# Nehliin/vortex

Measured on AMD Instinct MI355X. Metric: GiB/s SHA-1 piece hashing (device-resident), 256 KiB pieces, 1/2/4/8 MI355X, higher is better.
Workload: dtype u32; 1 GPU; 65536 x 256 KiB pieces per GPU (BASELINE config 2; config 4 at N=8), SHA-1 + verify vs expected table; pieces_per_gpu=65536, piece_len=262144, parallelism=piece-index shard x1, parity_checked=65536, parity_bit_exact=64881

## Files before the change

### include/vx_tuning.h

```cpp
#ifndef VX_TUNING_H
#define VX_TUNING_H
#include <stddef.h>
#include <stdint.h>
#ifndef VX_MERKLE_ASYNC_FUSED
#define VX_MERKLE_ASYNC_FUSED 1
#endif

#ifdef __cplusplus
extern "C" {
#endif

int vx_sha1_device_ragged_variant(const void* d_base, const uint64_t* d_offsets, const uint32_t* d_lens,
                                  const uint32_t* d_order, uint32_t n, void* d_digests, const void* d_expected,
                                  void* d_matched, void* stream, int variant);
struct vx_ctx;
struct vx_split;
int vx_tuning_zero_copy_plan(uint32_t n, uint64_t total_len);
int vx_tuning_zero_copy_kernel(const uint64_t* d_srcs, const uint32_t* d_lens, uint32_t n, void* d_digests,
                               const void* d_expected, void* d_matched, int loader, void* stream);
int vx_tuning_zero_tail_kernel(const void* d_base, const uint64_t* d_tail_offs, const uint32_t* d_lens,
                               const uint32_t* d_pads, uint32_t n, uint64_t piece_length, const uint32_t* d_states,
                               void* d_digests, void* stream);
int vx_tuning_chunk_kernel(const void* d_base, const uint64_t* d_offsets, const uint32_t* d_lens, uint32_t n,
                           const uint32_t* d_pids, const uint64_t* d_poffs, const uint64_t* d_tlens,
                           uint32_t* d_states, void* d_digests, void* stream);
void vx_tuning_fail_submit_after(struct vx_ctx* ctx, int64_t k);
void vx_tuning_fail_launch_after(struct vx_ctx* ctx, int64_t k);
void vx_tuning_verify_copy_stream(struct vx_ctx* ctx, int mode);
void vx_tuning_stage_huge(struct vx_ctx* ctx, int on);
void vx_tuning_split_rules(struct vx_ctx* ctx, int one_round, uint64_t round_cap, int lag, int learn);
int vx_tuning_plan_ragged(uint32_t n, uint32_t max_len, uint64_t total_len);
size_t vx_tuning_chunk_schedule(uint64_t L, uint64_t C, int head, int tail, uint64_t* out, size_t max);
uint64_t vx_tuning_split_take_tail(struct vx_split* s, uint64_t k, uint64_t* was);
size_t vx_tuning_last_split(const struct vx_ctx* ctx, double* out, size_t max);

int vx_sha1_device_uniform_variant(const void* d_base, uint64_t stride, uint32_t len, uint32_t n, void* d_digests,
                                   const void* d_expected, void* d_matched, void* stream, int variant);

int vx_tuning_clock_stamp(void* d_out, uint32_t blocks, void* stream);
int vx_tuning_wall_clock_khz(int device);
int vx_tuning_device_identity(int device, char* bus_id, size_t len, char* uuid16);

#ifdef __cplusplus
}
#endif
#endif
```

### vortex_amd/_lib.py

```python
from __future__ import annotations

import ctypes
import os
import threading

_HERE = os.path.dirname(os.path.abspath(__file__))
LIB_PATH = os.path.join(_HERE, "libvortex_amd.so")
TUNING_PATH = os.path.join(_HERE, "libvortex_amd_tuning.so")

VX_OK = 0
VX_EINVAL = -22
VX_ENOMEM = -12
VX_ERANGE = -34
VX_ENODEV = -19
VX_EDEVICE = -5
VX_EBUSY = -16

VX_MERKLE_BLOCK = 16384
VX_SHA256_LEN = 32

EXPORTS = (
    "vx_abi_version", "vx_last_error", "vx_strerror", "vx_device_count", "vx_config_default",
    "vx_create", "vx_destroy", "vx_register_host_buffer", "vx_unregister_host_buffer",
    "vx_submit", "vx_flush", "vx_poll", "vx_drain", "vx_pending", "vx_set_piece_table", "vx_submit_piece",
    "vx_sha1_batch", "vx_verify_batch", "vx_verify_files", "vx_verify_files_range", "vx_verify_files_multi",
    "vx_sha1_device_uniform", "vx_sha1_device_ragged", "vx_sha1_device_ragged_hint", "vx_sort_order",
    "vx_plan_verify", "vx_plan_verify_gpus", "vx_plan_verify_split", "vx_get_stats", "vx_reset_stats",
    "vx_last_verify", "vx_last_verify_rounds",
    "vx_split_init", "vx_split_claim", "vx_split_done", "vx_split_boundary", "vx_verify_files_split",
    "vx_verify_files_split_multi",
    "vx_merkle_device_uniform", "vx_merkle_device_ragged", "vx_merkle_device_root", "vx_merkle_pad_hash",
    "vx_merkle_verify_batch",
    "vx_merkle_device_blocks", "vx_merkle_device_nodes", "vx_merkle_verify_files", "vx_merkle_verify_files_range",
    "vx_merkle_device_pieces", "vx_merkle_submit", "vx_merkle_poll",
    "vx_merkle_layers_plan", "vx_merkle_device_layers", "vx_merkle_device_proofs", "vx_merkle_verify_layers",
    "vx_merkle_verify_proofs",
    "vx_hybrid_device_pieces", "vx_hybrid_verify_files", "vx_hybrid_verify_files_range",
    "vx_hybrid_submit", "vx_hybrid_set_piece_tables", "vx_hybrid_submit_piece", "vx_hybrid_poll",
)
TUNING_EXPORTS = (
    "vx_synth_fill", "vx_sha1_device_uniform_variant", "vx_sha1_device_ragged_variant",
    "vx_tuning_zero_copy_plan", "vx_tuning_zero_copy_kernel", "vx_tuning_plan_ragged", "vx_tuning_chunk_schedule",
    "vx_tuning_fail_submit_after", "vx_tuning_fail_launch_after", "vx_tuning_verify_copy_stream", "vx_tuning_stage_huge",
    "vx_tuning_split_rules", "vx_tuning_clock_stamp",
    "vx_tuning_wall_clock_khz", "vx_tuning_device_identity", "vx_tuning_split_take_tail",
    "vx_tuning_last_split", "vx_tuning_zero_tail_kernel", "vx_tuning_chunk_kernel",
)


class VxError(RuntimeError):
    def __init__(self, code: int, where: str, msg: str):
        super().__init__(f"{where} failed: {code} ({msg})")
        self.code = code
        self.refused = None


class vx_completion(ctypes.Structure):
    _fields_ = [("tag", ctypes.c_uint64), ("matched", ctypes.c_uint8), ("digest", ctypes.c_uint8 * 20),
                ("_pad", ctypes.c_uint8 * 3)]


class vx_merkle_completion(ctypes.Structure):
    _fields_ = [("tag", ctypes.c_uint64), ("matched", ctypes.c_uint8), ("root", ctypes.c_uint8 * 32),
                ("_pad", ctypes.c_uint8 * 7)]


class vx_hybrid_completion(ctypes.Structure):
    _fields_ = [("tag", ctypes.c_uint64), ("matched", ctypes.c_uint8), ("_pad", ctypes.c_uint8 * 3),
                ("sha1", ctypes.c_uint8 * 20), ("root", ctypes.c_uint8 * 32)]


VX_MERKLE_TILE_ROWS = 512


class vx_merkle_tile(ctypes.Structure):
    _fields_ = [("in_row", ctypes.c_uint32), ("out", ctypes.c_uint32), ("rows", ctypes.c_uint16),
                ("levels", ctypes.c_uint8), ("last", ctypes.c_uint8), ("_pad", ctypes.c_uint32)]


class vx_merkle_layers_plan(ctypes.Structure):
    _fields_ = [("n_layers", ctypes.c_uint32), ("passes", ctypes.c_uint32), ("rows", ctypes.c_uint64),
                ("work_rows", ctypes.c_uint64), ("n_tiles", ctypes.c_uint32), ("pass_tiles", ctypes.c_uint32 * 4),
                ("_pad", ctypes.c_uint32)]


class vx_merkle_proof(ctypes.Structure):
    _fields_ = [("pos", ctypes.c_uint64), ("row", ctypes.c_uint32), ("expected", ctypes.c_uint32),
                ("span", ctypes.c_uint16), ("uncles", ctypes.c_uint8), ("_pad", ctypes.c_uint8 * 5)]


def proof_array(proofs):
    arr = (vx_merkle_proof * max(len(proofs), 1))()
    widths = (64, 32, 32, 16, 8)
    for i, p in enumerate(proofs):
        v = (p.pos, p.row, p.expected, p.span, p.uncles) if isinstance(p, vx_merkle_proof) else tuple(int(x) for x in p)
        if len(v) != 5 or any(not 0 <= x < 1 << w for x, w in zip(v, widths)):
            raise ValueError(f"proof {i}: (pos, row, expected, span, uncles) = {v} does not fit vx_merkle_proof")
        arr[i].pos, arr[i].row, arr[i].expected, arr[i].span, arr[i].uncles = v
    return arr


ABI_VERSION = 3

CONFIG_OPTIONS = ("zero_copy", "direct_io", "batch_chunk", "verify_chunk", "verify_cold_chunk", "verify_ramp",
                  "refuse_when_full")


class vx_config(ctypes.Structure):
    _fields_ = [("device", ctypes.c_int32), ("max_piece_len", ctypes.c_uint32), ("batch_pieces", ctypes.c_uint32),
                ("slots", ctypes.c_uint32), ("slot_bytes", ctypes.c_uint64)] + \
        [(name, ctypes.c_uint32) for name in CONFIG_OPTIONS]


class vx_plan(ctypes.Structure):
    _fields_ = [("gpu_s", ctypes.c_double), ("gpu_chain_s", ctypes.c_double), ("gpu_transfer_s", ctypes.c_double),
                ("cpu_s", ctypes.c_double), ("piece_latency_s", ctypes.c_double),
                ("cpu_piece_latency_s", ctypes.c_double), ("use_gpu", ctypes.c_int32), ("_pad", ctypes.c_uint32)]


VX_STATS_HIST = 24


class vx_stats(ctypes.Structure):
    _fields_ = [(name, ctypes.c_uint64) for name in (
        "pieces_completed", "pieces_mismatched", "bytes_completed", "batches", "chunk_rounds", "gather_tiles",
        "staged_bytes", "io_errors", "submit_stall_ns", "batch_latency_count", "batch_latency_sum_us",
        "batch_latency_max_us")] + [("batch_latency_hist", ctypes.c_uint64 * VX_STATS_HIST)] + [
        (name, ctypes.c_uint64) for name in ("zero_copy_slots", "zero_copy_loader_slots", "submits_refused")]


class vx_verify_trace(ctypes.Structure):
    _fields_ = [(name, ctypes.c_double) for name in (
        "wall_ms", "read_busy_ms", "read_span_ms", "first_read_ms", "copy_busy_ms", "copy_span_ms", "tail_ms")] + [
        ("read_bytes", ctypes.c_uint64), ("copy_bytes", ctypes.c_uint64), ("readers", ctypes.c_uint32),
        ("rounds", ctypes.c_uint32), ("direct_bytes", ctypes.c_uint64),
        ("chunk_bytes", ctypes.c_uint64)]


VX_ROUND_NEW_WINDOW, VX_ROUND_HEAD_RAMP, VX_ROUND_TAIL_RAMP = 1, 2, 4


class vx_verify_round(ctypes.Structure):
    _fields_ = [(name, ctypes.c_double) for name in (
        "read_submit_ms", "read_done_ms", "enqueue_ms", "copy_start_ms", "copy_end_ms", "kernel_end_ms")] + [
        ("bytes", ctypes.c_uint64), ("offset", ctypes.c_uint64), ("lanes", ctypes.c_uint32),
        ("flags", ctypes.c_uint32)]


class vx_split(ctypes.Structure):
    _fields_ = [("word", ctypes.c_uint64), ("pool_done", ctypes.c_uint64), ("start_ns", ctypes.c_uint64),
                ("first", ctypes.c_uint64), ("end", ctypes.c_uint64), ("cpu_threads", ctypes.c_uint32),
                ("engines", ctypes.c_uint32), ("cpu_thread_rate", ctypes.c_double),
                ("pool_last_ns", ctypes.c_uint64)]


_lib = None
_tuning = None
_lock = threading.Lock()


def _declare(L: ctypes.CDLL, tuning: bool = False) -> None:
    c = ctypes
    vp = c.c_void_p
    sig = {
        "vx_abi_version": ([], c.c_int),
        "vx_last_error": ([], c.c_char_p),
        "vx_strerror": ([c.c_int], c.c_char_p),
        "vx_device_count": ([], c.c_int),
        "vx_config_default": ([c.POINTER(vx_config), c.c_uint32], None),
        "vx_create": ([c.POINTER(vx_config), c.POINTER(vp)], c.c_int),
        "vx_destroy": ([vp], c.c_int),
        "vx_register_host_buffer": ([vp, vp, c.c_size_t], c.c_int),
        "vx_unregister_host_buffer": ([vp, vp], c.c_int),
        "vx_submit": ([vp, c.c_uint64, vp, c.c_uint32, vp], c.c_int),
        "vx_flush": ([vp], c.c_int),
        "vx_set_piece_table": ([vp, vp, c.c_uint32], c.c_int),
        "vx_submit_piece": ([vp, c.c_uint64, vp, c.c_uint32, c.c_uint32], c.c_int),
        "vx_poll": ([vp, c.POINTER(vx_completion), c.c_size_t], c.c_int64),
        "vx_drain": ([vp, c.c_uint32], c.c_int),
        "vx_pending": ([vp], c.c_uint64),
        "vx_get_stats": ([vp, c.POINTER(vx_stats)], c.c_int),
        "vx_reset_stats": ([vp], c.c_int),
        "vx_sha1_batch": ([vp, vp, vp, c.c_size_t, vp], c.c_int),
        "vx_verify_batch": ([vp, vp, vp, vp, c.c_size_t, vp, vp], c.c_int),
        "vx_verify_files": ([vp, vp, vp, c.c_size_t, c.c_uint32, vp, c.c_size_t, vp, c.c_uint32], c.c_int64),
        "vx_verify_files_range": ([vp, vp, vp, c.c_size_t, c.c_uint32, vp, c.c_size_t, c.c_size_t, c.c_size_t, vp,
                                   c.c_uint32], c.c_int64),
        "vx_verify_files_multi": ([vp, c.c_size_t, vp, vp, c.c_size_t, c.c_uint32, vp, c.c_size_t, vp, c.c_uint32],
                                  c.c_int64),
        "vx_sha1_device_uniform": ([vp, c.c_uint64, c.c_uint32, c.c_uint32, vp, vp, vp, vp], c.c_int),
        "vx_sha1_device_ragged": ([vp, vp, vp, vp, c.c_uint32, vp, vp, vp, vp], c.c_int),
        "vx_sha1_device_ragged_hint": ([vp, vp, vp, vp, c.c_uint32, c.c_uint32, c.c_uint64, vp, vp, vp, vp],
                                       c.c_int),
        "vx_sort_order": ([vp, c.c_uint32, vp], c.c_int),
        "vx_last_verify": ([vp, c.POINTER(vx_verify_trace)], c.c_int),
        "vx_last_verify_rounds": ([vp, c.POINTER(vx_verify_round), c.c_size_t], c.c_int64),
        "vx_plan_verify": ([c.c_uint64, c.c_uint32, c.c_uint64, c.c_uint32, c.c_double, c.POINTER(vx_plan)], c.c_int),
        "vx_plan_verify_gpus": ([c.c_uint64, c.c_uint32, c.c_uint64, c.c_uint32, c.c_double, c.c_uint32,
                                 c.POINTER(vx_plan)], c.c_int),
        "vx_plan_verify_split": ([c.c_uint64, c.c_uint32, c.c_uint64, c.c_uint32, c.c_double, c.c_uint32,
                                  c.POINTER(c.c_uint64), c.POINTER(c.c_uint64), c.POINTER(vx_plan)], c.c_int),
        "vx_split_init": ([c.POINTER(vx_split), c.c_uint64, c.c_uint64, c.c_uint32, c.c_double], c.c_int),
        "vx_split_claim": ([c.POINTER(vx_split)], c.c_int64),
        "vx_split_done": ([c.POINTER(vx_split), c.c_uint64], None),
        "vx_split_boundary": ([c.POINTER(vx_split)], c.c_uint64),
        "vx_verify_files_split": ([vp, vp, vp, c.c_size_t, c.c_uint32, vp, c.c_size_t, c.POINTER(vx_split), vp,
                                   c.c_uint32], c.c_int64),
        "vx_verify_files_split_multi": ([vp, c.c_size_t, vp, vp, c.c_size_t, c.c_uint32, vp, c.c_size_t,
                                         c.POINTER(vx_split), vp, c.c_uint32], c.c_int64),
        "vx_merkle_device_uniform": ([vp, c.c_uint64, c.c_uint32, c.c_uint32, c.c_uint32, c.c_uint32, vp, vp, vp, vp,
                                      vp], c.c_int),
        "vx_merkle_device_ragged": ([vp, vp, vp, vp, c.c_uint32, c.c_uint32, vp, vp, vp, vp, vp], c.c_int),
        "vx_merkle_device_root": ([vp, c.c_uint32, c.c_uint32, vp, vp, vp], c.c_int),
        "vx_merkle_pad_hash": ([c.c_uint32, vp], c.c_int),
        "vx_merkle_verify_batch": ([vp, vp, vp, vp, c.c_size_t, c.c_uint32, vp, vp, vp], c.c_int),
        "vx_merkle_device_blocks": ([vp, vp, vp, c.c_uint32, vp, vp], c.c_int),
        "vx_merkle_device_nodes": ([vp, vp, c.c_uint32, c.c_uint32, vp, vp, vp, vp], c.c_int),
        "vx_merkle_verify_files": ([vp, vp, vp, c.c_size_t, c.c_uint32, vp, c.c_size_t, vp, c.c_uint32], c.c_int64),
        "vx_merkle_verify_files_range": ([vp, vp, vp, c.c_size_t, c.c_uint32, vp, c.c_size_t, c.c_size_t,
                                          c.c_size_t, vp, c.c_uint32], c.c_int64),
        "vx_merkle_device_pieces": ([vp, vp, vp, vp, c.c_uint32, c.c_uint32, vp, vp, vp, vp, vp], c.c_int),
        "vx_merkle_submit": ([vp, c.c_uint64, vp, c.c_uint32, c.c_uint32, vp], c.c_int),
        "vx_merkle_poll": ([vp, c.POINTER(vx_merkle_completion), c.c_size_t], c.c_int64),
        "vx_merkle_layers_plan": ([vp, c.c_uint32, c.POINTER(vx_merkle_layers_plan), vp, c.c_size_t], c.c_int),
        "vx_merkle_device_layers": ([vp, c.POINTER(vx_merkle_layers_plan), vp, c.c_uint32, vp, vp, vp, vp, vp],
                                    c.c_int),
        "vx_merkle_device_proofs": ([vp, vp, c.c_uint32, vp, vp, vp, vp], c.c_int),
        "vx_merkle_verify_layers": ([vp, vp, vp, c.c_uint32, c.c_uint32, vp, vp, vp], c.c_int),
        "vx_merkle_verify_proofs": ([vp, vp, c.c_uint64, vp, c.c_uint32, vp, c.c_uint32, vp, vp], c.c_int),
        "vx_hybrid_device_pieces": ([vp, vp, vp, vp, vp, c.c_uint32, c.c_uint32, vp, vp, vp, vp, vp, vp, vp], c.c_int),
        "vx_hybrid_verify_files": ([vp, vp, vp, c.c_size_t, c.c_uint32, vp, vp, c.c_size_t, vp, c.c_uint32],
                                   c.c_int64),
        "vx_hybrid_verify_files_range": ([vp, vp, vp, c.c_size_t, c.c_uint32, vp, vp, c.c_size_t, c.c_size_t,
                                          c.c_size_t, vp, c.c_uint32], c.c_int64),
        "vx_hybrid_submit": ([vp, c.c_uint64, vp, c.c_uint32, c.c_uint32, c.c_uint32, vp, vp], c.c_int),
        "vx_hybrid_set_piece_tables": ([vp, vp, vp, c.c_uint32], c.c_int),
        "vx_hybrid_submit_piece": ([vp, c.c_uint64, vp, c.c_uint32, c.c_uint32, c.c_uint32, c.c_uint32], c.c_int),
        "vx_hybrid_poll": ([vp, c.POINTER(vx_hybrid_completion), c.c_size_t], c.c_int64),
    }
    if tuning:
        sig.update({
            "vx_sha1_device_uniform_variant": ([vp, c.c_uint64, c.c_uint32, c.c_uint32, vp, vp, vp, vp, c.c_int],
                                               c.c_int),
            "vx_sha1_device_ragged_variant": ([vp, vp, vp, vp, c.c_uint32, vp, vp, vp, vp, c.c_int], c.c_int),
            "vx_tuning_zero_copy_plan": ([c.c_uint32, c.c_uint64], c.c_int),
            "vx_tuning_zero_copy_kernel": ([vp, vp, c.c_uint32, vp, vp, vp, c.c_int, vp], c.c_int),
            "vx_tuning_zero_tail_kernel": ([vp, vp, vp, vp, c.c_uint32, c.c_uint64, vp, vp, vp], c.c_int),
            "vx_tuning_chunk_kernel": ([vp, vp, vp, c.c_uint32, vp, vp, vp, vp, vp, vp], c.c_int),
            "vx_tuning_fail_submit_after": ([vp, c.c_int64], None),
            "vx_tuning_fail_launch_after": ([vp, c.c_int64], None),
            "vx_tuning_verify_copy_stream": ([vp, c.c_int], None),
            "vx_tuning_stage_huge": ([vp, c.c_int], None),
            "vx_tuning_split_rules": ([vp, c.c_int, c.c_uint64, c.c_int, c.c_int], None),
            "vx_tuning_clock_stamp": ([vp, c.c_uint32, vp], c.c_int),
            "vx_tuning_wall_clock_khz": ([c.c_int], c.c_int),
            "vx_tuning_device_identity": ([c.c_int, c.c_char_p, c.c_size_t, c.c_char_p], c.c_int),
            "vx_tuning_plan_ragged": ([c.c_uint32, c.c_uint32, c.c_uint64], c.c_int),
            "vx_tuning_split_take_tail": ([c.POINTER(vx_split), c.c_uint64, c.POINTER(c.c_uint64)], c.c_uint64),
            "vx_tuning_last_split": ([vp, c.POINTER(c.c_double), c.c_size_t], c.c_size_t),
            "vx_tuning_chunk_schedule": ([c.c_uint64, c.c_uint64, c.c_int, c.c_int, c.POINTER(c.c_uint64),
                                          c.c_size_t], c.c_size_t),
            "vx_synth_fill": ([vp, c.c_uint64, c.c_uint32, c.c_uint32, c.c_uint64, c.c_uint64, c.c_uint32, vp],
                              c.c_int),
        })
    for name, (args, res) in sig.items():
        fn = getattr(L, name)
        fn.argtypes = args
        fn.restype = res


def _load(path: str, tuning: bool) -> ctypes.CDLL:
    import torch

    if not os.path.exists(path):
        raise ImportError(
            f"{path} is missing: the HIP engine is not built. Run "
            "`python -c 'import __graft_entry__ as g; g.build()'` (or `make -C vortex_amd/csrc`).")
    L = ctypes.CDLL(path)
    _declare(L, tuning)
    if L.vx_abi_version() != ABI_VERSION:
        raise ImportError(f"{os.path.basename(path)} ABI version mismatch")
    return L


def lib() -> ctypes.CDLL:
    global _lib
    if _lib is not None:
        return _lib
    with _lock:
        if _lib is None:
            _lib = _load(LIB_PATH, False)
    return _lib


def tuning() -> ctypes.CDLL:
    global _tuning
    if _tuning is not None:
        return _tuning
    with _lock:
        if _tuning is None:
            _tuning = _load(TUNING_PATH, True)
    return _tuning


def check(rc: int, where: str, L: ctypes.CDLL | None = None) -> int:
    if rc < 0:
        msg = (L or lib()).vx_last_error().decode(errors="replace")
        raise VxError(rc, where, msg)
    return rc
```

### vortex_amd/csrc/sha1_kernels.hip

```cpp
#include <hip/hip_runtime.h>

#include <algorithm>
#include <cstdlib>
#include <stdint.h>

#include "sha1_consumer_asm.inc"
#include "sha1_device.hpp"
#include "vx_kernels.h"

namespace vx {

__device__ __attribute__((aligned(128))) uint4 g_zero_line[32];

__device__ __forceinline__ void load_group(uint4 (&dst)[8], const uint4* src) {
#pragma unroll
    for (int k = 0; k < 8; ++k) dst[k] = src[k];
}

__device__ __forceinline__ void load_group_ordered(uint4 (&dst)[8], const uint4* src) {
    __builtin_amdgcn_sched_barrier(0);
#pragma unroll
    for (int k = 0; k < 4; ++k) dst[k] = src[k];
    __builtin_amdgcn_sched_barrier(0);
#pragma unroll
    for (int k = 4; k < 8; ++k) dst[k] = src[k];
    __builtin_amdgcn_sched_barrier(0);
}

__device__ __forceinline__ void compress_group(State& s, const uint4 (&g)[8]) {
    compress_le(s, g[0], g[1], g[2], g[3]);
    compress_le(s, g[4], g[5], g[6], g[7]);
}

template <int R, bool kUniform, bool kFence = false>
__device__ __forceinline__ void stream_groups(State& s, const uint4* src, uint32_t ng, uint32_t ng_wave) {
    if (ng_wave == 0) return;
    const uint4* base = ng ? src : g_zero_line;
    const uint32_t last = ng ? ng - 1 : 0;
    uint4 ring[R][8];
#pragma unroll
    for (int r = 0; r < R - 1; ++r) {
        const uint32_t g = (uint32_t)r < last ? (uint32_t)r : last;
        if (kFence && kUniform)
            load_group_ordered(ring[r], base + (size_t)g * 8);
        else
            load_group(ring[r], base + (size_t)g * 8);
    }
    if (kFence && kUniform) {
        uint32_t g0 = 0;
        for (; g0 + R <= ng_wave; g0 += R) {
#pragma unroll
            for (int r = 0; r < R; ++r) {
                const uint32_t gl_raw = g0 + r + R - 1;
                const uint32_t gl = gl_raw < last ? gl_raw : last;
                load_group_ordered(ring[(r + R - 1) % R], base + (size_t)gl * 8);
                compress_group(s, ring[r]);
            }
        }
#pragma unroll
        for (int r = 0; r < R - 1; ++r)
            if (g0 + r < ng_wave) compress_group(s, ring[r]);
        return;
    }
    for (uint32_t g0 = 0; g0 < ng_wave; g0 += R) {
#pragma unroll
        for (int r = 0; r < R; ++r) {
            const uint32_t gl_raw = g0 + r + R - 1;
            const uint32_t gl = gl_raw < last ? gl_raw : last;
            load_group(ring[(r + R - 1) % R], base + (size_t)gl * 8);
            if (kUniform) {
                if (g0 + r < ng_wave) compress_group(s, ring[r]);
            } else {
                if (g0 + r < ng) compress_group(s, ring[r]);
            }
        }
    }
}

template <bool kUniform, int R = kRing, bool kFence = false>
__device__ __forceinline__ void hash_piece(State& s, const uint8_t* p, uint32_t len, uint32_t ng_wave) {
    const uint32_t nfull = len >> 6;
    const uint32_t ng = nfull >> 1;
    stream_groups<R, kUniform, kFence>(s, reinterpret_cast<const uint4*>(p), ng, ng_wave);
    const uint8_t* q = p + (size_t)ng * 128;
    if (nfull & 1) {
        const uint4* q4 = reinterpret_cast<const uint4*>(q);
        compress_le(s, q4[0], q4[1], q4[2], q4[3]);
        q += 64;
    }
    finalize(s, q, len & 63u, len);
}

__device__ __forceinline__ void emit(const State& s, uint32_t idx, uint8_t* __restrict__ digests,
                                     const uint8_t* __restrict__ expected, uint8_t* __restrict__ matched,
                                     const uint32_t* __restrict__ exp_index = nullptr) {
    const uint32_t d0 = bswap(s.h0), d1 = bswap(s.h1), d2 = bswap(s.h2), d3 = bswap(s.h3), d4 = bswap(s.h4);
    if (digests) {
        uint32_t* o = reinterpret_cast<uint32_t*>(digests + (size_t)idx * 20);
        o[0] = d0;
        o[1] = d1;
        o[2] = d2;
        o[3] = d3;
        o[4] = d4;
    }
    if (expected && matched) {
        const uint32_t row = exp_index ? exp_index[idx] : idx;
        const uint32_t* x = reinterpret_cast<const uint32_t*>(expected + (size_t)row * 20);
        const bool ok = (x[0] == d0) & (x[1] == d1) & (x[2] == d2) & (x[3] == d3) & (x[4] == d4);
        matched[idx] = ok ? 1 : 0;
    }
}

__device__ __forceinline__ uint32_t wave_min(uint32_t v) {
#pragma unroll
    for (int o = 32; o > 0; o >>= 1) {
        const uint32_t u = __shfl_xor(v, o, 64);
        v = u < v ? u : v;
    }
    return v;
}

__device__ __forceinline__ uint32_t wave_max(uint32_t v) {
#pragma unroll
    for (int o = 32; o > 0; o >>= 1) {
        const uint32_t u = __shfl_xor(v, o, 64);
        v = u > v ? u : v;
    }
    return v;
}

template <int R, bool kAlias = false, bool kFence = false>
__global__ __launch_bounds__(kBlock) void sha1_uniform_kernel(const uint8_t* __restrict__ base, uint64_t stride,
                                                              uint32_t len, uint32_t n,
                                                              uint8_t* __restrict__ digests,
                                                              const uint8_t* __restrict__ expected,
                                                              uint8_t* __restrict__ matched,
                                                              const uint32_t* __restrict__ exp_index) {
    const uint32_t i = blockIdx.x * kBlock + threadIdx.x;
    const uint32_t pi = kAlias ? 0 : (i < n ? i : n - 1);
    State s = iv();
    hash_piece<true, R, kFence>(s, base + (size_t)pi * stride, len, (len >> 7));
    if (i < n) emit(s, i, digests, expected, matched, exp_index);
}

__global__ __launch_bounds__(kBlock) void sha1_ragged_kernel(const uint8_t* __restrict__ base,
                                                             const uint64_t* __restrict__ offsets,
                                                             const uint32_t* __restrict__ lens,
                                                             const uint32_t* __restrict__ order, uint32_t n,
                                                             uint8_t* __restrict__ digests,
                                                             const uint8_t* __restrict__ expected,
                                                             uint8_t* __restrict__ matched,
                                                             const uint32_t* __restrict__ exp_index) {
    const uint32_t j = blockIdx.x * kBlock + threadIdx.x;
    const uint32_t jj = j < n ? j : n - 1;
    const uint32_t idx = order ? order[jj] : jj;
    const uint32_t len = lens[idx];
    const uint8_t* p = base + offsets[idx];
    const uint32_t ng_wave = __builtin_amdgcn_readfirstlane(wave_max(len >> 7));
    State s = iv();
    hash_piece<false>(s, p, len, ng_wave);
    if (j < n) emit(s, idx, digests, expected, matched, exp_index);
}



__device__ __forceinline__ void expand_store(uint32_t (&w)[16], uint4 (*dst)[64], int lane) {
#pragma unroll
    for (int q = 0; q < 4; ++q) dst[q][lane] = make_uint4(w[4 * q], w[4 * q + 1], w[4 * q + 2], w[4 * q + 3]);
#pragma unroll
    for (int q = 4; q < 20; ++q) {
        uint32_t v[4];
#pragma unroll
        for (int j = 0; j < 4; ++j) {
            const int t = 4 * q + j;
            const uint32_t x = rotl(VX_XOR2(VX_PAR(w[(t - 3) & 15], w[(t - 8) & 15], w[(t - 14) & 15]), w[t & 15]), 1);
            w[t & 15] = x;
            v[j] = x;
        }
        dst[q][lane] = make_uint4(v[0], v[1], v[2], v[3]);
    }
}

__device__ __forceinline__ void rounds_lds(State& s, const uint4 (*src)[64], int lane) {
    uint32_t a = s.h0, b = s.h1, c = s.h2, d = s.h3, e = s.h4;
#pragma unroll
    for (int q = 0; q < 20; ++q) {
        const uint4 w4 = src[q][lane];
        const uint32_t wq[4] = {w4.x, w4.y, w4.z, w4.w};
#pragma unroll
        for (int j = 0; j < 4; ++j) {
            const int t = 4 * q + j;
            uint32_t f, k;
            if (t < 20) {
                f = VX_CH(b, c, d);
                k = kK0;
            } else if (t < 40) {
                f = VX_PAR(b, c, d);
                k = kK1;
            } else if (t < 60) {
                f = VX_MAJ(b, c, d);
                k = kK2;
            } else {
                f = VX_PAR(b, c, d);
                k = kK3;
            }
            const uint32_t tmp = rotl(a, 5) + f + e + k + wq[j];
            e = d;
            d = c;
            c = rotl(b, 30);
            b = a;
            a = tmp;
        }
    }
    s.h0 += a;
    s.h1 += b;
    s.h2 += c;
    s.h3 += d;
    s.h4 += e;
}

template <int S>
struct RingLds {
    uint4 w[S][20][64];
};

template <int S>
__device__ __forceinline__ uint32_t ring_slot(uint32_t b) {
    return S == 2 ? (b & 1u) : (b % 3u);
}

template <int S>
__device__ __forceinline__ void publish(uint32_t b) {
    if (S == 2 || b >= 1) __syncthreads();
}

template <int S>
__device__ __forceinline__ void producer_done(uint32_t nb_wave) {
    if (S == 2) {
        __syncthreads();
    } else if (nb_wave) {
        __syncthreads();
        __syncthreads();
    }
}

__device__ __forceinline__ void load_w(uint4 (&r)[20], const uint4 (*src)[64], int lane) {
#pragma unroll
    for (int q = 0; q < 20; ++q) r[q] = src[q][lane];
}

__device__ __forceinline__ void rounds_regs(State& s, const uint4 (&w)[20]) {
    uint32_t a = s.h0, b = s.h1, c = s.h2, d = s.h3, e = s.h4;
#pragma unroll
    for (int q = 0; q < 20; ++q) {
        const uint32_t wq[4] = {w[q].x, w[q].y, w[q].z, w[q].w};
#pragma unroll
        for (int j = 0; j < 4; ++j) {
            const int t = 4 * q + j;
            uint32_t f, k;
            if (t < 20) {
                f = VX_CH(b, c, d);
                k = kK0;
            } else if (t < 40) {
                f = VX_PAR(b, c, d);
                k = kK1;
            } else if (t < 60) {
                f = VX_MAJ(b, c, d);
                k = kK2;
            } else {
                f = VX_PAR(b, c, d);
                k = kK3;
            }
            const uint32_t tmp = rotl(a, 5) + f + e + k + wq[j];
            e = d;
            d = c;
            c = rotl(b, 30);
            b = a;
            a = tmp;
        }
    }
    s.h0 += a;
    s.h1 += b;
    s.h2 += c;
    s.h3 += d;
    s.h4 += e;
}

template <bool kSelect>
__device__ __forceinline__ void consume_asm(State& s, const uint4* lds_lane, uint32_t nb_wave, uint32_t b1,
                                            uint32_t nb) {
    const uint32_t addr = (uint32_t)(uintptr_t)lds_lane;
    if (kSelect)
        asm volatile(VX_CONSUMER_SELECT_ASM
                     : "+v"(s.h0), "+v"(s.h1), "+v"(s.h2), "+v"(s.h3), "+v"(s.h4)
                     : "v"(addr), "s"(nb_wave), "s"(b1), "v"(nb)
                     : VX_CONSUMER_SELECT_ASM_CLOBBERS, "memory");
    else
        asm volatile(VX_CONSUMER_ASM
                     : "+v"(s.h0), "+v"(s.h1), "+v"(s.h2), "+v"(s.h3), "+v"(s.h4)
                     : "v"(addr), "s"(nb_wave), "s"(b1), "v"(nb)
                     : VX_CONSUMER_ASM_CLOBBERS, "memory");
}

template <int S, bool kSelect>
__device__ __forceinline__ void consume(State& s, RingLds<S>& lds, int lane, uint32_t nb_wave, uint32_t b1,
                                        uint32_t nb) {
    if (S == 2) {
        __syncthreads();
        for (uint32_t b = 0; b < b1; ++b) {
            rounds_lds(s, lds.w[b & 1], lane);
            __syncthreads();
        }
        if (kSelect) {
            for (uint32_t b = b1; b < nb_wave; ++b) {
                State t = s;
                rounds_lds(t, lds.w[b & 1], lane);
                if (b < nb) s = t;
                __syncthreads();
            }
        }
        return;
    }
#ifndef VX_CONSUMER_CC
    if (S == 3) {
        consume_asm<kSelect>(s, &lds.w[0][0][lane], nb_wave, b1, nb);
        return;
    }
#endif
    if (nb_wave == 0) return;
    auto step = [&](uint32_t b, const uint4 (&r)[20]) {
        if (!kSelect || b < b1) {
            rounds_regs(s, r);
        } else {
            State t = s;
            rounds_regs(t, r);
            if (b < nb) s = t;
        }
        asm volatile("" : "+v"(s.h0), "+v"(s.h1), "+v"(s.h2), "+v"(s.h3), "+v"(s.h4));
    };
    uint4 r0[20], r1[20];
    __syncthreads();
    load_w(r0, lds.w[0], lane);
    __builtin_amdgcn_s_waitcnt(0xC07F);
    uint32_t b = 0;
    for (; b + 2 <= nb_wave; b += 2) {
        load_w(r1, lds.w[ring_slot<S>(b + 1)], lane);
        __builtin_amdgcn_sched_barrier(0);
        step(b, r0);
        __builtin_amdgcn_sched_barrier(0);
        __syncthreads();
        if (b + 2 < nb_wave) load_w(r0, lds.w[ring_slot<S>(b + 2)], lane);
        __builtin_amdgcn_sched_barrier(0);
        step(b + 1, r1);
        __builtin_amdgcn_sched_barrier(0);
        __syncthreads();
    }
    if (b < nb_wave) {
        step(b, r0);
        __builtin_amdgcn_sched_barrier(0);
        __syncthreads();
    }
}

__device__ __forceinline__ void le_words(uint32_t (&w)[16], const uint4& q0, const uint4& q1, const uint4& q2,
                                         const uint4& q3) {
    const uint4 q[4] = {q0, q1, q2, q3};
#pragma unroll
    for (int k = 0; k < 4; ++k) {
        w[4 * k + 0] = bswap(q[k].x);
        w[4 * k + 1] = bswap(q[k].y);
        w[4 * k + 2] = bswap(q[k].z);
        w[4 * k + 3] = bswap(q[k].w);
    }
}

__device__ __forceinline__ void tail_words(uint32_t (&w)[16], const uint8_t* q, uint32_t rem) {
    const uint32_t* q32 = reinterpret_cast<const uint32_t*>(q);
#pragma unroll
    for (int k = 0; k < 16; ++k) {
        const uint32_t off = 4u * k;
        uint32_t v = 0;
        if (off + 4 <= rem) {
            v = q32[k];
        } else if (off < rem) {
            for (uint32_t j = 0; off + j < rem; ++j) v |= (uint32_t)q[off + j] << (8 * j);
        }
        if (rem >= off && rem < off + 4) v |= 0x80u << (8 * (rem - off));
        w[k] = bswap(v);
    }
}

template <int S>
__global__ __launch_bounds__(kPairBlock) void sha1_split_kernel(const uint8_t* __restrict__ base, uint64_t stride,
                                                                uint32_t len, uint32_t n,
                                                                uint8_t* __restrict__ digests,
                                                                const uint8_t* __restrict__ expected,
                                                                uint8_t* __restrict__ matched,
                                                                const uint32_t* __restrict__ exp_index) {
    __shared__ RingLds<S> lds;
    const int lane = threadIdx.x & 63;
    const int wave = __builtin_amdgcn_readfirstlane(threadIdx.x >> 6);
    const uint32_t i = blockIdx.x * 64 + lane;
    const uint32_t pi = i < n ? i : n - 1;
    const uint8_t* p = base + (size_t)pi * stride;
    const uint32_t nfull = len >> 6;
    const uint32_t rem = len & 63u;
    const uint32_t nb = nfull + (rem <= 55 ? 1u : 2u);

    if (wave == 1) {
        uint32_t b = 0;
        uint32_t w[16];
        const uint32_t ng = len >> 7;
        const uint4* src = reinterpret_cast<const uint4*>(p);
        if (ng) {
            constexpr int R = kRing;
            const uint32_t last = ng - 1;
            uint4 ring[R][8];
#pragma unroll
            for (int r = 0; r < R - 1; ++r) {
                const uint32_t g = (uint32_t)r < last ? (uint32_t)r : last;
                load_group(ring[r], src + (size_t)g * 8);
            }
            for (uint32_t g0 = 0; g0 < ng; g0 += R) {
#pragma unroll
                for (int r = 0; r < R; ++r) {
                    const uint32_t gl_raw = g0 + r + R - 1;
                    const uint32_t gl = gl_raw < last ? gl_raw : last;
                    load_group(ring[(r + R - 1) % R], src + (size_t)gl * 8);
                    if (g0 + r < ng) {
                        le_words(w, ring[r][0], ring[r][1], ring[r][2], ring[r][3]);
                        expand_store(w, lds.w[ring_slot<S>(b)], lane);
                        publish<S>(b);
                        ++b;
                        le_words(w, ring[r][4], ring[r][5], ring[r][6], ring[r][7]);
                        expand_store(w, lds.w[ring_slot<S>(b)], lane);
                        publish<S>(b);
                        ++b;
                    }
                }
            }
        }
        const uint8_t* q = p + (size_t)ng * 128;
        if (nfull & 1) {
            const uint4* q4 = reinterpret_cast<const uint4*>(q);
            le_words(w, q4[0], q4[1], q4[2], q4[3]);
            expand_store(w, lds.w[ring_slot<S>(b)], lane);
            publish<S>(b);
            ++b;
            q += 64;
        }
        tail_words(w, q, rem);
        const uint32_t bits_hi = (uint32_t)(((uint64_t)len * 8u) >> 32);
        const uint32_t bits_lo = (uint32_t)((uint64_t)len * 8u);
        if (rem <= 55) {
            w[14] = bits_hi;
            w[15] = bits_lo;
            expand_store(w, lds.w[ring_slot<S>(b)], lane);
            publish<S>(b);
        } else {
            expand_store(w, lds.w[ring_slot<S>(b)], lane);
            publish<S>(b);
            ++b;
#pragma unroll
            for (int k = 0; k < 14; ++k) w[k] = 0;
            w[14] = bits_hi;
            w[15] = bits_lo;
            expand_store(w, lds.w[ring_slot<S>(b)], lane);
            publish<S>(b);
        }
        producer_done<S>(nb);
    } else {
        State s = iv();
        consume<S, false>(s, lds, lane, nb, nb, nb);
        if (i < n) emit(s, i, digests, expected, matched, exp_index);
    }
}

template <int S>
hipError_t launch_uniform_split_s(const uint8_t* base, uint64_t stride, uint32_t len, uint32_t n, uint8_t* digests,
                                  const uint8_t* expected, uint8_t* matched, hipStream_t stream,
                                  const uint32_t* exp_index) {
    const uint32_t blocks = (n + 63) / 64;
    hipLaunchKernelGGL(sha1_split_kernel<S>, dim3(blocks), dim3(kPairBlock), 0, stream, base, stride, len, n,
                       digests, expected, matched, exp_index);
    return hipGetLastError();
}

hipError_t launch_uniform_split(const uint8_t* base, uint64_t stride, uint32_t len, uint32_t n, uint8_t* digests,
                                const uint8_t* expected, uint8_t* matched, hipStream_t stream,
                                const uint32_t* exp_index) {
    return launch_uniform_split_s<kSplitSlots>(base, stride, len, n, digests, expected, matched, stream, exp_index);
}


constexpr int kBlockRing = 6;

__device__ __forceinline__ void load_block(uint4 (&dst)[4], const uint4* src) {
#pragma unroll
    for (int k = 0; k < 4; ++k) dst[k] = src[k];
}

__device__ __forceinline__ void pad_words(uint32_t (&w)[16], const uint8_t* q, uint32_t rem, uint64_t len,
                                          uint32_t k) {
    const uint32_t bits_hi = (uint32_t)((len * 8u) >> 32);
    const uint32_t bits_lo = (uint32_t)(len * 8u);
    if (k == 0) {
        tail_words(w, q, rem);
        if (rem <= 55) {
            w[14] = bits_hi;
            w[15] = bits_lo;
        }
    } else {
#pragma unroll
        for (int j = 0; j < 16; ++j) w[j] = 0;
        if (k == 1 && rem > 55) {
            w[14] = bits_hi;
            w[15] = bits_lo;
        }
    }
}

template <bool kChunked, int S>
__global__ __launch_bounds__(kPairBlock) void sha1_ragged_split_kernel(
    const uint8_t* __restrict__ base, const uint64_t* __restrict__ offsets, const uint32_t* __restrict__ lens,
    const uint32_t* __restrict__ order, uint32_t n, uint8_t* __restrict__ digests,
    const uint8_t* __restrict__ expected, uint8_t* __restrict__ matched, const uint32_t* __restrict__ exp_index,
    const uint32_t* __restrict__ pids, const uint64_t* __restrict__ poffs, const uint64_t* __restrict__ tlens,
    uint32_t* __restrict__ states) {
    __shared__ RingLds<S> lds;
    const int lane = threadIdx.x & 63;
    const int wave = __builtin_amdgcn_readfirstlane(threadIdx.x >> 6);
    const uint32_t j = blockIdx.x * 64 + lane;
    const uint32_t jj = j < n ? j : n - 1;
    const uint32_t idx = order ? order[jj] : jj;
    const uint32_t len = lens[idx];
    const uint8_t* p = base + offsets[idx];
    const uint32_t pid = kChunked ? pids[idx] : idx;
    const uint64_t poff = kChunked ? poffs[idx] : 0;
    const uint64_t tlen = kChunked ? tlens[idx] : len;
    const bool final_chunk = poff + len == tlen;
    const uint32_t nfull = len >> 6;
    const uint32_t rem = len & 63u;
    const uint32_t nb = final_chunk ? nfull + (rem <= 55 ? 1u : 2u) : nfull;
    const uint32_t nb_wave = __builtin_amdgcn_readfirstlane(wave_max(nb));
    constexpr int R = kBlockRing;
    const uint32_t nfull_min = __builtin_amdgcn_readfirstlane(wave_min(nfull));
    const uint32_t b1 = nfull_min / R * R;

    if (wave == 1) {
        const uint4* src = nfull ? reinterpret_cast<const uint4*>(p) : g_zero_line;
        const uint32_t last = nfull ? nfull - 1 : 0;
        const uint8_t* q = p + (size_t)nfull * 64;
        uint32_t w[16];
        if (b1) {
            uint4 ring[R][4];
#pragma unroll
            for (int r = 0; r < R - 1; ++r) {
                __builtin_amdgcn_sched_barrier(0);
                load_block(ring[r], src + (size_t)r * 4);
            }
            for (uint32_t b0 = 0; b0 < b1; b0 += R) {
#pragma unroll
                for (int r = 0; r < R; ++r) {
                    const uint32_t bl_raw = b0 + r + R - 1;
                    const uint32_t bl = bl_raw < last ? bl_raw : last;
                    __builtin_amdgcn_sched_barrier(0);
                    load_block(ring[(r + R - 1) % R], src + (size_t)bl * 4);
                    __builtin_amdgcn_sched_barrier(0);
                    le_words(w, ring[r][0], ring[r][1], ring[r][2], ring[r][3]);
                    expand_store(w, lds.w[ring_slot<S>(b0 + r)], lane);
                    publish<S>(b0 + r);
                }
            }
        }
        if (b1 < nb_wave) {
            uint32_t padw[16];
            tail_words(padw, q, rem);
            const uint32_t bits_hi = (uint32_t)((tlen * 8u) >> 32);
            const uint32_t bits_lo = (uint32_t)(tlen * 8u);
            if (rem <= 55) {
                padw[14] = bits_hi;
                padw[15] = bits_lo;
            }
            uint4 ring[R][4];
#pragma unroll
            for (int r = 0; r < R - 1; ++r) {
                const uint32_t bl_raw = b1 + r;
                const uint32_t bl = bl_raw < last ? bl_raw : last;
                __builtin_amdgcn_sched_barrier(0);
                load_block(ring[r], src + (size_t)bl * 4);
            }
            for (uint32_t b0 = b1; b0 < nb_wave; b0 += R) {
#pragma unroll
                for (int r = 0; r < R; ++r) {
                    const uint32_t b = b0 + r;
                    const uint32_t bl_raw = b + R - 1;
                    const uint32_t bl = bl_raw < last ? bl_raw : last;
                    __builtin_amdgcn_sched_barrier(0);
                    load_block(ring[(r + R - 1) % R], src + (size_t)bl * 4);
                    __builtin_amdgcn_sched_barrier(0);
                    if (b < nb_wave) {
                        le_words(w, ring[r][0], ring[r][1], ring[r][2], ring[r][3]);
                        const bool is_pad0 = b == nfull;
                        const bool is_pad1 = b == nfull + 1;
#pragma unroll
                        for (int k = 0; k < 16; ++k) {
                            uint32_t v = b < nfull ? w[k] : 0u;
                            v = is_pad0 ? padw[k] : v;
                            if (k >= 14) v = (is_pad1 && rem > 55) ? (k == 14 ? bits_hi : bits_lo) : v;
                            w[k] = v;
                        }
                        expand_store(w, lds.w[ring_slot<S>(b)], lane);
                        publish<S>(b);
                    }
                }
            }
        }
        producer_done<S>(nb_wave);
    } else {
        State s = iv();
        if (kChunked && poff != 0) {
            const uint32_t* st = states + (size_t)pid * 5;
            s = State{st[0], st[1], st[2], st[3], st[4]};
        }
        consume<S, true>(s, lds, lane, nb_wave, b1, nb);
        if (j < n) {
            if (!kChunked || final_chunk) {
                emit(s, pid, digests, expected, matched, exp_index);
            } else {
                uint32_t* st = states + (size_t)pid * 5;
                st[0] = s.h0;
                st[1] = s.h1;
                st[2] = s.h2;
                st[3] = s.h3;
                st[4] = s.h4;
            }
        }
    }
}

constexpr uint32_t kWidePadLds = 40 * 1024;

template <int S>
hipError_t launch_ragged_split_s(const uint8_t* base, const uint64_t* offsets, const uint32_t* lens,
                                 const uint32_t* order, uint32_t n, uint8_t* digests, const uint8_t* expected,
                                 uint8_t* matched, hipStream_t stream, const uint32_t* exp_index,
                                 bool wide = false) {
    const uint32_t blocks = (n + 63) / 64;
    hipLaunchKernelGGL((sha1_ragged_split_kernel<false, S>), dim3(blocks), dim3(kPairBlock),
                       wide ? kWidePadLds : 0u, stream, base,
                       offsets, lens, order, n, digests, expected, matched, exp_index, nullptr, nullptr, nullptr,
                       nullptr);
    return hipGetLastError();
}

hipError_t launch_ragged_split(const uint8_t* base, const uint64_t* offsets, const uint32_t* lens,
                               const uint32_t* order, uint32_t n, uint8_t* digests, const uint8_t* expected,
                               uint8_t* matched, hipStream_t stream, const uint32_t* exp_index) {
    return launch_ragged_split_s<kSplitSlots>(base, offsets, lens, order, n, digests, expected, matched, stream,
                                              exp_index);
}

hipError_t launch_chunk(const uint8_t* base, const uint64_t* offsets, const uint32_t* lens, uint32_t n,
                        const uint32_t* pids, const uint64_t* poffs, const uint64_t* tlens, uint32_t* states,
                        uint8_t* digests, const uint8_t* expected, uint8_t* matched, hipStream_t stream) {
    if (n == 0) return hipSuccess;
    const uint32_t blocks = (n + 63) / 64;
    hipLaunchKernelGGL((sha1_ragged_split_kernel<true, kSplitSlots>), dim3(blocks), dim3(kPairBlock), 0, stream, base, offsets,
                       lens, nullptr, n, digests, expected, matched, nullptr, pids, poffs, tlens, states);
    return hipGetLastError();
}

constexpr uint32_t kZcPieces = 32;
constexpr uint32_t kZcTileBlocks = 8;
constexpr uint32_t kZcChunks = kZcTileBlocks * 4;

typedef uint32_t U32x4 __attribute__((ext_vector_type(4)));
typedef const __attribute__((address_space(1))) U32x4 GlobalU32x4;

__device__ __forceinline__ uint4 zc_load(int k, const uint64_t (&zb)[8], const uint32_t (&zl)[8], uint32_t t) {
    const uint32_t o = t * (kZcTileBlocks * 64) + (k >= 8 ? 256u : 0u);
    const uint64_t zero = reinterpret_cast<uint64_t>(g_zero_line);
    const uint64_t a = (o < zl[k & 7] ? zb[k & 7] + t * (kZcTileBlocks * 64) : zero) + (k >= 8 ? 256u : 0u);
    const U32x4 v = *reinterpret_cast<GlobalU32x4*>(a);
    return make_uint4(v.x, v.y, v.z, v.w);
}

__device__ __forceinline__ void zc_load_tile(uint4 (&r)[16], const uint64_t (&zb)[8], const uint32_t (&zl)[8],
                                             uint32_t t) {
#pragma unroll
    for (int k = 0; k < 16; ++k) r[k] = zc_load(k, zb, zl, t);
}

__device__ __forceinline__ void zc_load_pair(uint4 (&r)[16], int k0, const uint64_t (&zb)[8],
                                             const uint32_t (&zl)[8], uint32_t t) {
    r[k0] = zc_load(k0, zb, zl, t);
    r[k0 + 1] = zc_load(k0 + 1, zb, zl, t);
}

__device__ __forceinline__ void zc_setup(uint64_t (&zb)[8], uint32_t (&zl)[8], uint4 (&ra)[16], uint4 (&rb)[16],
                                         uint4 (&stage)[2][kZcChunks][kZcPieces + 1], const uint64_t* srcs,
                                         const uint32_t* lens, uint32_t n, uint32_t g0, int lane) {
    const uint32_t c16 = lane & 15;
#pragma unroll
    for (int g = 0; g < 8; ++g) {
        const uint32_t pk = g0 + 4 * g + (lane >> 4);
        const uint32_t pkk = pk < n ? pk : n - 1;
        const uint32_t full = pk < n ? (lens[pkk] >> 6) * 64u : 0u;
        zb[g] = srcs[pkk] + 16 * c16;
        zl[g] = full >= 16 * c16 + 16 ? full - 16 * c16 - 15 : 0u;
    }
    zc_load_tile(ra, zb, zl, 0);
    zc_load_tile(rb, zb, zl, 1);
#pragma unroll
    for (int k = 0; k < 16; ++k) {
        const uint32_t p = 4 * (k & 7) + (lane >> 4), c = c16 + 16 * (k >> 3);
        stage[0][c][p] = ra[k];
    }
    zc_load_tile(ra, zb, zl, 2);
}

template <int S, bool kLoader>
__global__ __launch_bounds__(kLoader ? 3 * 64 : kPairBlock) void sha1_zc_split_kernel(
    const uint64_t* __restrict__ srcs, const uint32_t* __restrict__ lens, uint32_t n, uint8_t* __restrict__ digests,
    const uint8_t* __restrict__ expected, uint8_t* __restrict__ matched, const uint32_t* __restrict__ exp_index) {
    __shared__ RingLds<S> lds;
    __shared__ uint4 stage[2][kZcChunks][kZcPieces + 1];
    __shared__ uint4 padl[4][64];
    const int lane = threadIdx.x & 63;
    const uint32_t pl = lane & (kZcPieces - 1);
    const int wave = __builtin_amdgcn_readfirstlane(threadIdx.x >> 6);
    const uint32_t g0 = blockIdx.x * kZcPieces;
    const uint32_t j = g0 + pl;
    const uint32_t jj = j < n ? j : n - 1;
    const uint32_t len = lens[jj];
    const uint32_t nfull = len >> 6;
    const uint32_t rem = len & 63u;
    const uint32_t nb = nfull + (rem <= 55 ? 1u : 2u);
    const uint32_t nb_wave = __builtin_amdgcn_readfirstlane(wave_max(nb));
    const uint32_t c16 = lane & 15;
    const uint32_t ntiles = (nb_wave + kZcTileBlocks - 1) / kZcTileBlocks;

#define VX_ZC_TILE(REG, T, RD, SEL, LOADS, HASH)                                                        \
    {                                                                                                   \
        const uint32_t t = (T);                                                                         \
        _Pragma("unroll") for (uint32_t bb = 0; bb < kZcTileBlocks; ++bb) {                             \
            if (LOADS) {                                                                                \
                _Pragma("unroll") for (int k = 2 * bb; k < 2 * (int)bb + 2; ++k) {                      \
                    const uint32_t p = 4 * (k & 7) + (lane >> 4), c = c16 + 16 * (k >> 3);              \
                    stage[1 - (RD)][c][p] = REG[k];                                                     \
                }                                                                                       \
                zc_load_pair(REG, 2 * bb, zb, zl, t + 3);                                               \
            }                                                                                           \
            const uint32_t b = kZcTileBlocks * t + bb;                                                  \
            if ((HASH) && b < nb_wave) {                                              \
                const uint4 q0 = stage[RD][4 * bb + 0][pl];                                           \
                const uint4 q1 = stage[RD][4 * bb + 1][pl];                                           \
                const uint4 q2 = stage[RD][4 * bb + 2][pl];                                           \
                const uint4 q3 = stage[RD][4 * bb + 3][pl];                                           \
                le_words(w, q0, q1, q2, q3);                                                            \
                if (SEL) {                                                                              \
                    const uint4 p0 = padl[0][lane], p1 = padl[1][lane], p2 = padl[2][lane], p3 = padl[3][lane]; \
                    const uint32_t pw[16] = {p0.x, p0.y, p0.z, p0.w, p1.x, p1.y, p1.z, p1.w,            \
                                             p2.x, p2.y, p2.z, p2.w, p3.x, p3.y, p3.z, p3.w};           \
                    const bool is_pad0 = b == nfull;                                                    \
                    const bool is_pad1 = b == nfull + 1;                                                \
                    _Pragma("unroll") for (int k = 0; k < 16; ++k) {                                    \
                        uint32_t v = b < nfull ? w[k] : 0u;                                             \
                        v = is_pad0 ? pw[k] : v;                                                        \
                        if (k >= 14) v = (is_pad1 && rem > 55) ? (k == 14 ? bits_hi : bits_lo) : v;     \
                        w[k] = v;                                                                       \
                    }                                                                                   \
                }                                                                                       \
                expand_store(w, lds.w[ring_slot<S>(b)], lane);                                          \
            }                                                                                           \
               \
                    \
            if (b < nb_wave) publish<S>(b);                                                             \
        }                                                                                               \
    }
    if (wave == 0) {
        const uint32_t b1 = __builtin_amdgcn_readfirstlane(wave_min(nb));
        State s = iv();
        if (kLoader) __syncthreads();
        consume<S, true>(s, lds, lane, nb_wave, b1, nb);
        if (lane < (int)kZcPieces && j < n) emit(s, j, digests, expected, matched, exp_index);
    } else if (kLoader && wave == 2) {
        uint64_t zb[8];
        uint32_t zl[8];
        uint4 ra[16], rb[16];
        uint32_t w[16];
        const uint32_t bits_hi = 0, bits_lo = 0;
        zc_setup(zb, zl, ra, rb, stage, srcs, lens, n, g0, lane);
        __syncthreads();
        for (uint32_t t0 = 0; t0 < ntiles; t0 += 2) {
            VX_ZC_TILE(rb, t0, 0, 0, 1, 0)
            VX_ZC_TILE(ra, t0 + 1, 1, 0, 1, 0)
        }
        (void)w;
        (void)bits_hi;
        (void)bits_lo;
        producer_done<S>(nb_wave);
    } else {
        uint32_t padw[16];
        const uint8_t* q = reinterpret_cast<const uint8_t*>(srcs[jj]) + (size_t)nfull * 64;
        tail_words(padw, q, rem);
        const uint32_t bits_hi = (uint32_t)(((uint64_t)len * 8u) >> 32);
        const uint32_t bits_lo = (uint32_t)((uint64_t)len * 8u);
        if (rem <= 55) {
            padw[14] = bits_hi;
            padw[15] = bits_lo;
        }
#pragma unroll
        for (int k = 0; k < 4; ++k) padl[k][lane] = make_uint4(padw[4 * k], padw[4 * k + 1], padw[4 * k + 2], padw[4 * k + 3]);
        const uint32_t b_sel = __builtin_amdgcn_readfirstlane(wave_min(nfull));
        uint64_t zb[8];
        uint32_t zl[8];
        uint4 ra[16], rb[16];
        uint32_t w[16];
        if (kLoader)
            __syncthreads();
        else
            zc_setup(zb, zl, ra, rb, stage, srcs, lens, n, g0, lane);
        for (uint32_t t0 = 0; t0 < ntiles; t0 += 2) {
            if (kZcTileBlocks * (t0 + 1) <= b_sel) VX_ZC_TILE(rb, t0, 0, 0, !kLoader, 1) else VX_ZC_TILE(rb, t0, 0, 1, !kLoader, 1)
            if (kZcTileBlocks * (t0 + 2) <= b_sel) VX_ZC_TILE(ra, t0 + 1, 1, 0, !kLoader, 1) else VX_ZC_TILE(ra, t0 + 1, 1, 1, !kLoader, 1)
        }
        producer_done<S>(nb_wave);
    }
#undef VX_ZC_TILE
}

hipError_t launch_zero_copy(const uint64_t* srcs, const uint32_t* lens, uint32_t n, uint8_t* digests,
                            const uint8_t* expected, uint8_t* matched, bool loader, hipStream_t stream,
                            const uint32_t* exp_index) {
    if (n == 0) return hipSuccess;
    const uint32_t blocks = (n + kZcPieces - 1) / kZcPieces;
    if (loader)
        hipLaunchKernelGGL((sha1_zc_split_kernel<kSplitSlots, true>), dim3(blocks), dim3(3 * 64), 0, stream, srcs,
                           lens, n, digests, expected, matched, exp_index);
    else
        hipLaunchKernelGGL((sha1_zc_split_kernel<kSplitSlots, false>), dim3(blocks), dim3(kPairBlock), 0, stream,
                           srcs, lens, n, digests, expected, matched, exp_index);
    return hipGetLastError();
}

template <int R, bool kAlias = false, bool kFence = false>
hipError_t launch_uniform_lane_r(const uint8_t* base, uint64_t stride, uint32_t len, uint32_t n, uint8_t* digests,
                                 const uint8_t* expected, uint8_t* matched, hipStream_t stream,
                                 const uint32_t* exp_index) {
    const uint32_t blocks = (n + kBlock - 1) / kBlock;
    hipLaunchKernelGGL((sha1_uniform_kernel<R, kAlias, kFence>), dim3(blocks), dim3(kBlock), 0, stream, base, stride, len, n, digests,
                       expected, matched, exp_index);
    return hipGetLastError();
}

hipError_t launch_uniform_lane(const uint8_t* base, uint64_t stride, uint32_t len, uint32_t n, uint8_t* digests,
                               const uint8_t* expected, uint8_t* matched, hipStream_t stream,
                               const uint32_t* exp_index) {
    return launch_uniform_lane_r<kLaneRing, false, true>(base, stride, len, n, digests, expected, matched, stream,
                                                         exp_index);
}

hipError_t launch_ragged_lane(const uint8_t* base, const uint64_t* offsets, const uint32_t* lens,
                              const uint32_t* order, uint32_t n, uint8_t* digests, const uint8_t* expected,
                              uint8_t* matched, hipStream_t stream, const uint32_t* exp_index) {
    const uint32_t blocks = (n + kBlock - 1) / kBlock;
    hipLaunchKernelGGL(sha1_ragged_kernel, dim3(blocks), dim3(kBlock), 0, stream, base, offsets, lens, order, n,
                       digests, expected, matched, exp_index);
    return hipGetLastError();
}

}

namespace vx {
hipError_t launch_uniform(const uint8_t* base, uint64_t stride, uint32_t len, uint32_t n, uint8_t* digests,
                          const uint8_t* expected, uint8_t* matched, hipStream_t stream, int variant,
                          const uint32_t* exp_index) {
    if (variant == kUniformLane) return launch_uniform_lane(base, stride, len, n, digests, expected, matched, stream, exp_index);
    if (variant == kUniformSplit) return launch_uniform_split(base, stride, len, n, digests, expected, matched, stream, exp_index);
    if (variant == kSplitRing2)
        return launch_uniform_split_s<2>(base, stride, len, n, digests, expected, matched, stream, exp_index);
    if (variant == kSplitRing3)
        return launch_uniform_split_s<3>(base, stride, len, n, digests, expected, matched, stream, exp_index);
    if (n <= kSplitMaxPieces) return launch_uniform_split(base, stride, len, n, digests, expected, matched, stream, exp_index);
    return launch_uniform_lane(base, stride, len, n, digests, expected, matched, stream, exp_index);
}
}

namespace vx {
int plan_ragged(uint32_t n, uint64_t max_len, uint64_t total_len) {
    (void)n;
    const double blocks = (double)((max_len + 9 + 63) / 64);
    const double lane = std::max((double)total_len / 3.4e12, blocks * 1.18e-6);
    const double split = std::max((double)total_len / 2.5e12, blocks * 0.77e-6);
    if (lane < split) return kUniformLane;
    return (double)total_len / 1.25e12 <= 0.5 * blocks * 0.77e-6 ? kSplitWide : kUniformSplit;
}

hipError_t launch_ragged(const uint8_t* base, const uint64_t* offsets, const uint32_t* lens, const uint32_t* order,
                         uint32_t n, uint8_t* digests, const uint8_t* expected, uint8_t* matched,
                         hipStream_t stream, int variant, const uint32_t* exp_index) {
    if (variant == kUniformLane) return launch_ragged_lane(base, offsets, lens, order, n, digests, expected, matched, stream, exp_index);
    if (variant == kSplitRing2)
        return launch_ragged_split_s<2>(base, offsets, lens, order, n, digests, expected, matched, stream, exp_index);
    if (variant == kSplitRing3)
        return launch_ragged_split_s<3>(base, offsets, lens, order, n, digests, expected, matched, stream, exp_index);
    if (variant == kSplitWide)
        return launch_ragged_split_s<kSplitSlots>(base, offsets, lens, order, n, digests, expected, matched, stream,
                                                  exp_index, true);
    return launch_ragged_split(base, offsets, lens, order, n, digests, expected, matched, stream, exp_index);
}
}
```

Measured before the change: 3343 GiB/s.

## Switch SHA-1 LDS consumer to phased inline-asm loop; add optional chain stamps

By default the kernel now includes a new phased consumer assembly file and passes a rounded-down count of whole unrolled blocks to it, instead of the previous burst consumer. This changes how LDS loads and SHA-1 rounds are interleaved in the hot loop, aiming to hide LDS latency behind the dependency chain. The old consumer stays available under VX_CONSUMER_BURST. A compile-time VX_CHAIN_STAMPS path and a host API record per-block timestamps for profiling. The new asm file is not shown, so correctness of its remainder handling cannot be checked here.

```diff
diff --git a/include/vx_tuning.h b/include/vx_tuning.h
--- a/include/vx_tuning.h
+++ b/include/vx_tuning.h
@@ -38,6 +38,7 @@
                                    const void* d_expected, void* d_matched, void* stream, int variant);
 
 int vx_tuning_clock_stamp(void* d_out, uint32_t blocks, void* stream);
+int vx_tuning_chain_log(void* d_log, uint32_t blocks, uint32_t cap);
 int vx_tuning_wall_clock_khz(int device);
 int vx_tuning_device_identity(int device, char* bus_id, size_t len, char* uuid16);
 
diff --git a/vortex_amd/_lib.py b/vortex_amd/_lib.py
--- a/vortex_amd/_lib.py
+++ b/vortex_amd/_lib.py
@@ -42,7 +42,7 @@
     "vx_synth_fill", "vx_sha1_device_uniform_variant", "vx_sha1_device_ragged_variant",
     "vx_tuning_zero_copy_plan", "vx_tuning_zero_copy_kernel", "vx_tuning_plan_ragged", "vx_tuning_chunk_schedule",
     "vx_tuning_fail_submit_after", "vx_tuning_fail_launch_after", "vx_tuning_verify_copy_stream", "vx_tuning_stage_huge",
-    "vx_tuning_split_rules", "vx_tuning_clock_stamp",
+    "vx_tuning_split_rules", "vx_tuning_clock_stamp", "vx_tuning_chain_log",
     "vx_tuning_wall_clock_khz", "vx_tuning_device_identity", "vx_tuning_split_take_tail",
     "vx_tuning_last_split", "vx_tuning_zero_tail_kernel", "vx_tuning_chunk_kernel",
 )
@@ -253,6 +253,7 @@
             "vx_tuning_stage_huge": ([vp, c.c_int], None),
             "vx_tuning_split_rules": ([vp, c.c_int, c.c_uint64, c.c_int, c.c_int], None),
             "vx_tuning_clock_stamp": ([vp, c.c_uint32, vp], c.c_int),
+            "vx_tuning_chain_log": ([vp, c.c_uint32, c.c_uint32], c.c_int),
             "vx_tuning_wall_clock_khz": ([c.c_int], c.c_int),
             "vx_tuning_device_identity": ([c.c_int, c.c_char_p, c.c_size_t, c.c_char_p], c.c_int),
             "vx_tuning_plan_ragged": ([c.c_uint32, c.c_uint32, c.c_uint64], c.c_int),
diff --git a/vortex_amd/csrc/sha1_kernels.hip b/vortex_amd/csrc/sha1_kernels.hip
--- a/vortex_amd/csrc/sha1_kernels.hip
+++ b/vortex_amd/csrc/sha1_kernels.hip
@@ -4,13 +4,25 @@
 #include <cstdlib>
 #include <stdint.h>
 
+#ifdef VX_CONSUMER_BURST
 #include "sha1_consumer_asm.inc"
+#else
+#include "sha1_consumer_phased_asm.inc"
+#endif
+#ifdef VX_CHAIN_STAMPS
+#include "sha1_consumer_stamps_asm.inc"
+#endif
 #include "sha1_device.hpp"
 #include "vx_kernels.h"
 
 namespace vx {
 
 __device__ __attribute__((aligned(128))) uint4 g_zero_line[32];
+
+#ifdef VX_CHAIN_STAMPS
+__device__ uint4* g_chain_log = nullptr;
+__device__ uint32_t g_chain_cap = 0, g_chain_blocks = 0;
+#endif
 
 __device__ __forceinline__ void load_group(uint4 (&dst)[8], const uint4* src) {
 #pragma unroll
@@ -290,6 +302,33 @@
 __device__ __forceinline__ void consume_asm(State& s, const uint4* lds_lane, uint32_t nb_wave, uint32_t b1,
                                             uint32_t nb) {
     const uint32_t addr = (uint32_t)(uintptr_t)lds_lane;
+#ifndef VX_CONSUMER_BURST
+    const uint32_t whole = b1 / VX_CONSUMER_UNROLL * VX_CONSUMER_UNROLL;
+#ifdef VX_CHAIN_STAMPS
+    if (kSelect) {
+        const bool on = g_chain_log && blockIdx.x < g_chain_blocks;
+        const uint32_t cap = __builtin_amdgcn_readfirstlane(on ? g_chain_cap : 0u);
+        const uint64_t at = (uint64_t)(uintptr_t)(g_chain_log + (size_t)blockIdx.x * cap);
+        asm volatile(VX_CONSUMER_STAMPED_SELECT_ASM
+                     : "+v"(s.h0), "+v"(s.h1), "+v"(s.h2), "+v"(s.h3), "+v"(s.h4)
+                     : "v"(addr), "s"(nb_wave), "s"(whole), "v"(nb), "v"((uint32_t)at), "v"((uint32_t)(at >> 32)),
+                       "s"(cap)
+                     : VX_CONSUMER_STAMPED_SELECT_ASM_CLOBBERS, "memory");
+        return;
+    }
+#endif
+    if (kSelect)
+        asm volatile(VX_CONSUMER_PHASED_SELECT_ASM
+                     : "+v"(s.h0), "+v"(s.h1), "+v"(s.h2), "+v"(s.h3), "+v"(s.h4)
+                     : "v"(addr), "s"(nb_wave), "s"(whole), "v"(nb)
+                     : VX_CONSUMER_PHASED_SELECT_ASM_CLOBBERS, "memory");
+    else
+        asm volatile(VX_CONSUMER_PHASED_ASM
+                     : "+v"(s.h0), "+v"(s.h1), "+v"(s.h2), "+v"(s.h3), "+v"(s.h4)
+                     : "v"(addr), "s"(nb_wave), "s"(whole), "v"(nb)
+                     : VX_CONSUMER_PHASED_ASM_CLOBBERS, "memory");
+    return;
+#else
     if (kSelect)
         asm volatile(VX_CONSUMER_SELECT_ASM
                      : "+v"(s.h0), "+v"(s.h1), "+v"(s.h2), "+v"(s.h3), "+v"(s.h4)
@@ -300,6 +339,7 @@
                      : "+v"(s.h0), "+v"(s.h1), "+v"(s.h2), "+v"(s.h3), "+v"(s.h4)
                      : "v"(addr), "s"(nb_wave), "s"(b1), "v"(nb)
                      : VX_CONSUMER_ASM_CLOBBERS, "memory");
+#endif
 }
 
 template <int S, bool kSelect>
@@ -912,3 +952,20 @@
     return launch_ragged_split(base, offsets, lens, order, n, digests, expected, matched, stream, exp_index);
 }
 }
+
+extern "C" int vx_tuning_chain_log(void* d_log, uint32_t blocks, uint32_t cap) {
+#ifdef VX_CHAIN_STAMPS
+    if (d_log && (blocks == 0 || cap < 2 || (reinterpret_cast<uintptr_t>(d_log) & 15))) return -22;
+    if (hipDeviceSynchronize() != hipSuccess) return -5;
+    uint4* p = static_cast<uint4*>(d_log);
+    const uint32_t b = d_log ? blocks : 0, c = d_log ? cap : 0;
+    if (hipMemcpyToSymbol(HIP_SYMBOL(vx::g_chain_cap), &c, sizeof c) != hipSuccess ||
+        hipMemcpyToSymbol(HIP_SYMBOL(vx::g_chain_blocks), &b, sizeof b) != hipSuccess ||
+        hipMemcpyToSymbol(HIP_SYMBOL(vx::g_chain_log), &p, sizeof p) != hipSuccess)
+        return -5;
+    return 0;
+#else
+    (void)d_log, (void)blocks, (void)cap;
+    return -22;
+#endif
+}
```

New measurement: 3350 GiB/s, median of 2. About the same (+0.2%).
